# glennhickey/teHmm

Measured on AMD Instinct MI355X. Metric: genome positions/sec (Viterbi+posterior), 35 states x 10 tracks, higher is better.
Workload: dtype f64

## Files before the change

### tehmm_amd/csrc/tehmm_fused.hip.h

```cpp
#pragma once
#include "tehmm_lane.hip.h"

namespace tehmm {

template <int NT>
struct FusedGeom {
  static constexpr int KS = NT / 4;
  static constexpr int KSP = ((KS + 1) + 1) & ~1;
  static constexpr int RT = (NT + 15) / 16;
  static constexpr int SLICE_B = KSP * 8;
  static constexpr int ROW_D = 4 * KSP;
  static constexpr int ROW_D_LDS = 4 * KSP + 2;
};

#ifndef TEHMM_FUSED_2W
#define TEHMM_FUSED_2W 36
#endif
#define TEHMM_FUSED_BLKW 24
#ifndef TEHMM_FUSED_NSLOT_CAP
#define TEHMM_FUSED_NSLOT_CAP 64
#endif

struct FusedTab {
  const unsigned long long *rixx;
// ... 213 lines not shown
    const int blk = e / fo.SB, r = e - blk * fo.SB;
    unsigned long long *dst = rixx + ((tile * fo.NB + blk) * TEHMM_FUSED_BLKW + (int64_t)r * fo.FKW) * 16 + i16;
    for (int w = 0; w < fo.FKW; ++w) {
      unsigned long long word = 0;
      for (int b = 0; b < 4; ++b) {
        const int i = 4 * w + b;
        int v = 0;
        if (i < fo.K) {
          const int sym = orow[fo.order[i]];
          v = sym < fo.cnt[i] ? fo.base[i] + sym : (i < fo.n_glb ? fo.zero_glb : fo.zero_lds);
        }
        word |= (unsigned long long)(v & 0xffff) << (16 * b);
      }
      dst[(int64_t)w * 16] = word;
    }
  }
}


#define TEHMM_RIX_CB 4
#define TEHMM_RIX_STG 129
template <int FKW>
__global__ __launch_bounds__(256) void k_fused_rowindex(IntervalTab iv, LaneGeom lg, FusedOrder fo, const uint8_t *obs,
                                                        unsigned long long *rixx, int cps) {
  constexpr int SB = TEHMM_FUSED_BLKW / FKW, CB = TEHMM_RIX_CB, NS = CB * SB, STG = TEHMM_RIX_STG;
  __shared__ fused_u4 s_img[CB * 192];
  __shared__ fused_u4 s_slot[2 * TEHMM_FUSED_BLKW];
  __shared__ unsigned s_obs[16 * STG];
  __shared__ long long s_a0[16], s_T[16], s_row0[16];
  const int tid = threadIdx.x, lane = tid & 63, wv = tid >> 6;
  const int64_t tile = blockIdx.x;
  const int KPW = fo.KP >> 2;
  if (tid < 4 * TEHMM_FUSED_BLKW) {
    unsigned x = 0, y = 0;
    if (tid < fo.K) {
      const int cnt = fo.cnt[tid] < 256 ? fo.cnt[tid] : 256;
      x = (unsigned)fo.order[tid] | ((unsigned)cnt << 8);
      y = ((unsigned)fo.base[tid] & 0xffffu) | ((unsigned)(tid < fo.n_glb ? fo.zero_glb : fo.zero_lds) << 16);
    }
    unsigned *sl = (unsigned *)s_slot;
    sl[2 * tid] = x;
    sl[2 * tid + 1] = y;
  } else if (tid >= 128 && tid < 144) {
    const int64_t item = tile * 16 + (tid - 128);
    const bool valid = item < lg.n_items;
    const int id = valid ? lg.item_iv[item] : 0;
    s_a0[tid - 128] = (valid ? lg.item_t0[item] : 0) - fo.Wu;
    s_T[tid - 128] = iv.len[id];
    s_row0[tid - 128] = iv.pos0[id];
  }
  __syncthreads();
  const int nchunk = (fo.NB + CB - 1) / CB;
  const int c0 = blockIdx.y * cps, c1 = min(c0 + cps, nchunk);
  auto clampT = [](int64_t t, int64_t T) { return T > 0 ? (t < 0 ? 0 : (t >= T ? T - 1 : t)) : 0; };
  unsigned rr[4][2];
  auto load = [&](int c) {
#pragma unroll
    for (int j = 0; j < 4; ++j) {
      const int it = wv * 4 + j;
      const int64_t a = s_a0[it] + (int64_t)c * NS, T = s_T[it];
      const int64_t tf = clampT(a, T), tl = clampT(a + NS - 1, T);
      const int nd = (int)(tl - tf + 1) * KPW;
      const unsigned *src = (const unsigned *)obs + (s_row0[it] + tf) * KPW;
#pragma unroll
      for (int k = 0; k < 2; ++k) rr[j][k] = lane + 64 * k < nd ? src[lane + 64 * k] : 0u;
    }
  };
  const int i16 = tid & 15, q = tid >> 4;
  const int64_t my_a0 = s_a0[i16], my_T = s_T[i16];
  if (c0 < c1) load(c0);
  for (int c = c0; c < c1; ++c) {
#pragma unroll
    for (int j = 0; j < 4; ++j) {
#pragma unroll
      for (int k = 0; k < 2; ++k) s_obs[(wv * 4 + j) * STG + lane + 64 * k] = rr[j][k];
    }
    __syncthreads();
    if (c + 1 < c1) load(c + 1);
    const int64_t a = my_a0 + (int64_t)c * NS;
    int lo = 0, hi = 0, off = 0;
    if (my_T > 0) {
      const int64_t big = 1 << 30, l = -a, h = my_T - 1 - a;
      lo = (int)(l < -big ? -big : (l > big ? big : l));
      hi = (int)(h < -big ? -big : (h > big ? big : h));
      off = (int)(a - clampT(a, my_T));
    }
    const uint8_t *stage = (const uint8_t *)s_obs + i16 * (STG * 4);
#pragma unroll
    for (int jj = 0; jj < CB * TEHMM_FUSED_BLKW / 16; ++jj) {
      const int sw = q + 16 * jj, step = sw / FKW, w = sw - step * FKW;
      const uint8_t *row = stage + (min(max(step, lo), hi) + off) * fo.KP;
      const fused_u4 sa = s_slot[2 * w], sb = s_slot[2 * w + 1];
      const unsigned sx[4] = {sa.x, sa.z, sb.x, sb.z}, sy[4] = {sa.y, sa.w, sb.y, sb.w};
      unsigned long long word = 0;
#pragma unroll
      for (int b = 0; b < 4; ++b) {
        const unsigned sym = row[sx[b] & 0xffu];
        const unsigned v = sym < (sx[b] >> 8) ? (sy[b] & 0xffffu) + sym : sy[b] >> 16;
        word |= (unsigned long long)(v & 0xffffu) << (16 * b);
      }
      ((unsigned long long *)s_img)[tid + 256 * jj] = word;
    }
    __syncthreads();
    fused_u4 *dst = (fused_u4 *)rixx + (tile * fo.NB + (int64_t)c * CB) * 192;
#pragma unroll
    for (int jj = 0; jj < CB * 192 / 256; ++jj) {
      const int p = tid + 256 * jj;
      if (c * CB + p / 192 < fo.NB) dst[p] = s_img[p];
    }
  }
}

template <int NT, bool LOGDOM>
__global__ __launch_bounds__(256) __attribute__((amdgpu_waves_per_eu(NT <= TEHMM_FUSED_2W ? 2 : 1, NT <= TEHMM_FUSED_2W ? 2 : 1)))
void k_fused_fwd(IntervalTab iv, FusedTab ft, LaneGeom lg, int N, int CS, int Wu,
                 const double *__restrict__ tab , float *al32, double *chkf, double *pre,
                 double *end, double *slog32) {
  using G = FusedGeom<NT>;
  constexpr int KS = G::KS, RT = G::RT;
  extern __shared__ double fused_lds[];
  fused_stage<NT>(ft, fused_lds);
  __syncthreads();
  const int lane = threadIdx.x & 63;
  const int tile = blockIdx.x * 4 + (threadIdx.x >> 6);
  if (tile >= lg.n_groups * 4) return;
  const int L = lg.L;
  const int kq = lane >> 4;
  const int64_t item = (int64_t)tile * 16 + (lane & 15);
  const bool valid = item < lg.n_items;
  const int id = valid ? lg.item_iv[item] : 0;
  const int64_t t0 = valid ? lg.item_t0[item] : 0;
  const int64_t T = iv.len[id];
  const int64_t ct0 = (t0 / CS) * CS;
  const bool run = valid && ct0 + CS <= T && ct0 > 0;
  if (!__any(run)) return;
  double tf[RT][KS];
#pragma unroll
  for (int rt = 0; rt < RT; ++rt) {
#pragma unroll
    for (int s = 0; s < KS; ++s) {
      const int j = 16 * rt + (lane & 15), k = 4 * s + kq;
      tf[rt][s] = (j < NT) ? tab[k * NT + j] : 0.0;
    }
  }
  double v[KS];
#pragma unroll
  for (int s = 0; s < KS; ++s) v[s] = (kq + 4 * s < N) ? 1.0 / (double)N : 0.0;
  double slog = 0.0;
  auto vec_out = [&](double *dst) {
    const int64_t po = ((((item >> 6) * NT) + kq) << 6) + (item & 63);
#pragma unroll
    for (int s = 0; s < KS; ++s) dst[po + ((int64_t)(4 * s) << 6)] = v[s];
  };
  const double qnan = __longlong_as_double(0x7ff8000000000000LL);
  IndexWindow win;
  win.src = (const fused_u4 *)ft.rixx + (int64_t)tile * ft.NB * 192;
  win.lds_base = (unsigned)(size_t)(__attribute__((address_space(3))) const double *)fused_lds +
                 (unsigned)(ft.lds_rows * G::ROW_D_LDS * 8 + (threadIdx.x >> 6) * 2 * 3072);
  win.lane = lane;
  win.dir = 1;
  win.NB = ft.NB;
  win.start(0);
  double q[KS], ms;
  EmisStream<NT, LOGDOM> es(ft, fused_lds, win, kq);
  es.begin(0);
#pragma unroll
  for (int k = 0; k < KS; ++k) es.slot(k);
  es.finish(N, q, ms);
  const int E1 = ft.NB * ft.SB - 1;
  es.begin(min(1, E1));
  {
    float2 *ar = (float2 *)al32 + al32_index<NT>(lg, item, 0, kq) / 2;
#pragma unroll
    for (int p = 0; p < (KS + 1) / 2; ++p) ar[(int64_t)p * 64] = make_float2(0.f, 0.f);
  }
#ifdef TEHMM_STAMPS
  unsigned long long stq[4] = {0, 0, 0, 0}, stt = stamp_now();
#define FST(i) do { const unsigned long long n_ = stamp_now(); stq[i] += n_ - stt; stt = n_; } while (0)
#else
#define FST(i)
#endif
  for (int s = -Wu; s < L; ++s) {
    if (s == 0) {
      if (run) vec_out(pre);
      slog = 0.0;
    }
    FST(3);
    lane_d4 acc[RT];
#pragma unroll
    for (int rt = 0; rt < RT; ++rt) acc[rt] = (lane_d4){0.0, 0.0, 0.0, 0.0};
#pragma unroll
    for (int k = 0; k < KS; ++k) {
#pragma unroll
      for (int rt = 0; rt < RT; ++rt) acc[rt] = __builtin_amdgcn_mfma_f64_16x16x4f64(tf[rt][k], v[k], acc[rt], 0, 0, 0);
      es.slot(k);
      __builtin_amdgcn_sched_barrier(0);
    }
    FST(0);
    double qn[KS], msn = 0.0;
    es.finish(N, qn, msn);
    FST(1);
    double a[KS];
    double t = 0.0;
#pragma unroll
    for (int k = 0; k < KS; ++k) {
      a[k] = acc[k >> 2][k & 3] * q[k];
      t += a[k];
    }
    t = item_sum4(t);
    const int e = ((__double2hiint(t) >> 20) & 0x7ff) - 1022;
    const bool okrow = t > 1e-280 && t < INFINITY;
    const double scale = okrow ? __hiloint2double((1023 - e) << 20, 0) : qnan;
#pragma unroll
    for (int k = 0; k < KS; ++k) v[k] = a[k] * scale;
    slog += (double)e * 0.6931471805599453 + ms;
#pragma unroll
    for (int k = 0; k < KS; ++k) q[k] = qn[k];
    const double ms_now = ms;
    ms = msn;
    (void)ms_now;
    es.begin(min(s + 2 + Wu, E1));
    FST(2);
    {
      float2 *ar = (float2 *)al32 + al32_index<NT>(lg, item, s < 0 ? 0 : s, kq) / 2;
#pragma unroll
      for (int p = 0; p < (KS + 1) / 2; ++p)
        ar[(int64_t)p * 64] = run ? make_float2((float)v[2 * p], 2 * p + 1 < KS ? (float)v[2 * p + 1] : 0.f)
                                  : make_float2(0.f, 0.f);
    }
    if (s >= 0 && run) {
      if ((s & 31) == 31) {
        if (kq == 0) slog32[item * (L / 32) + (s >> 5)] = slog;
        if ((s & 63) == 31) {
          double *cr = chkf + (item * (L / 64) + (s >> 6)) * NT + kq;
#pragma unroll
          for (int k = 0; k < KS; ++k) cr[4 * k] = v[k];
        }
      }
    }
  }
  if (run) vec_out(end);
#ifdef TEHMM_STAMPS
  if (lane == 0 && blockIdx.x < 4096)
    for (int i = 0; i < 4; ++i) g_stamps[(blockIdx.x * 4 + (threadIdx.x >> 6)) * 4 + i] = stq[i];
#endif
#undef FST
}

template <int NT, bool LOGDOM, bool EPS, bool ESTEP = false>
__global__ __launch_bounds__(256) __attribute__((amdgpu_waves_per_eu(NT <= TEHMM_FUSED_2W ? 2 : 1, NT <= TEHMM_FUSED_2W ? 2 : 1)))
void k_fused_bwd(IntervalTab iv, FusedTab ft, LaneGeom lg, int N, int CS, int Wu,
                 const double *__restrict__ tab , const float *__restrict__ al32,
                 double *post, double *pre, double *end, double *chk, float *gam32 = nullptr, float *wz32 = nullptr,
                 double *sink = nullptr ) {
  using G = FusedGeom<NT>;
  constexpr int KS = G::KS, RT = G::RT;
  extern __shared__ double fused_lds[];
  fused_stage<NT>(ft, fused_lds);
  __syncthreads();
  const int lane = threadIdx.x & 63;
  const int tile = blockIdx.x * 4 + (threadIdx.x >> 6);
  if (tile >= lg.n_groups * 4) return;
  const int L = lg.L;
  const int kq = lane >> 4;
  const int64_t item = (int64_t)tile * 16 + (lane & 15);
  const bool valid = item < lg.n_items;
  const int id = valid ? lg.item_iv[item] : 0;
  const int64_t t0 = valid ? lg.item_t0[item] : 0;
  const int64_t T = iv.len[id];
  const int64_t ct0 = (t0 / CS) * CS;
  const bool run = valid && ct0 + CS <= T && ct0 + CS < T;
  if (!__any(run)) return;
  const int wu = !run ? 0 : (int)min((int64_t)Wu, T - (t0 + L));
  double tf[RT][KS];
#pragma unroll
  for (int rt = 0; rt < RT; ++rt) {
#pragma unroll
    for (int s = 0; s < KS; ++s) {
      const int j = 16 * rt + (lane & 15), k = 4 * s + kq;
      tf[rt][s] = (j < NT) ? tab[j * NT + k] : 0.0;
    }
  }
  double v[KS];
#pragma unroll
  for (int s = 0; s < KS; ++s) v[s] = 0.0;
  const int64_t prow0 = (iv.out0[id] + t0) * N;
  auto vec_out = [&](double *dst) {
    const int64_t po = ((((item >> 6) * NT) + kq) << 6) + (item & 63);
#pragma unroll
    for (int s = 0; s < KS; ++s) dst[po + ((int64_t)(4 * s) << 6)] = v[s];
  };
  const double eps = 1.1920928955078125e-07;
  const double inv_epsden = 1.0 / (1.0 + (double)N * eps);
  const double qnan = __longlong_as_double(0x7ff8000000000000LL);
  const int top = L + wu - 1;
  IndexWindow win;
  win.src = (const fused_u4 *)ft.rixx + (int64_t)tile * ft.NB * 192;
  win.lds_base = (unsigned)(size_t)(__attribute__((address_space(3))) const double *)fused_lds +
                 (unsigned)(ft.lds_rows * G::ROW_D_LDS * 8 + (threadIdx.x >> 6) * 2 * 3072);
  win.lane = lane;
  win.dir = -1;
  win.NB = ft.NB;
  win.start((L + 2 * Wu - 1) / ft.SB);
  typedef __attribute__((address_space(3))) double lds_f64;
  typedef __attribute__((address_space(3))) long long lds_i64;
  const unsigned ptile = (unsigned)(size_t)(__attribute__((address_space(3))) const double *)fused_lds +
                         (unsigned)(ft.lds_rows * G::ROW_D_LDS * 8 + 4 * 2 * 3072 + (threadIdx.x >> 6) * (16 * NT * 8 + 128));
  const unsigned pinfo = ptile + 16 * NT * 8;
  if (!ESTEP && kq == 0) *(lds_i64 *)(size_t)(pinfo + (lane & 15) * 8) = run ? (long long)prow0 : -1ll;
  double q[KS], ms;
  EmisStream<NT, LOGDOM> es(ft, fused_lds, win, kq);
  es.begin(L + 2 * Wu - 1);
#pragma unroll
  for (int k = 0; k < KS; ++k) es.slot(k);
  es.finish(N, q, ms);
  es.begin(max(L + 2 * Wu - 2, 0));
#ifdef TEHMM_STAMPS
  unsigned long long stq[4] = {0, 0, 0, 0}, stt = stamp_now();
#define FST(i) do { const unsigned long long n_ = stamp_now(); stq[i] += n_ - stt; stt = n_; } while (0)
#else
#define FST(i)
#endif
  for (int s = L + Wu - 1; s >= 0; --s) {
    if (s == L - 1 && run) vec_out(pre);
    FST(3);
    lane_d4 acc[RT];
#pragma unroll
    for (int rt = 0; rt < RT; ++rt) acc[rt] = (lane_d4){0.0, 0.0, 0.0, 0.0};
    float2 alp[(KS + 1) / 2];
    {
      const float2 *ar = (const float2 *)al32 + al32_index<NT>(lg, item, s < L ? s : L - 1, kq) / 2;
#pragma unroll
      for (int p = 0; p < (KS + 1) / 2; ++p) alp[p] = ar[(int64_t)p * 64];
    }
#pragma unroll
    for (int k = 0; k < KS; ++k) {
#pragma unroll
      for (int rt = 0; rt < RT; ++rt) acc[rt] = __builtin_amdgcn_mfma_f64_16x16x4f64(tf[rt][k], v[k], acc[rt], 0, 0, 0);
      es.slot(k);
      __builtin_amdgcn_sched_barrier(0);
    }
    FST(0);
#pragma unroll
    for (int p = 0; p < (KS + 1) / 2; ++p) asm volatile("" : "+v"(alp[p].x), "+v"(alp[p].y));
#pragma unroll
    for (int p = 0; p < (KS + 1) / 2; ++p) alp[p] = run ? alp[p] : make_float2(0.f, 0.f);
    double qn[KS], msn = 0.0;
    es.finish(N, qn, msn);
    FST(1);
    double t = 0.0;
#pragma unroll
    for (int k = 0; k < KS; ++k) t += acc[k >> 2][k & 3];
    t = item_sum4(t);
    const int e = ((__double2hiint(t) >> 20) & 0x7ff) - 1022;
    double bt[KS];
    const bool okrow = (s >= L && s >= top) || (t > 0.0 && t < INFINITY);
    const double scale = okrow ? __hiloint2double((1023 - e) << 20, 0) : qnan;
#pragma unroll
    for (int k = 0; k < KS; ++k) {
      bt[k] = acc[k >> 2][k & 3] * scale;
      if (s >= L && s == top) bt[k] = kq + 4 * k < N ? 1.0 : 0.0;
    }
    double g[KS];
    float wzf[ESTEP ? KS : 1];
#pragma unroll
    for (int k = 0; k < KS; ++k) g[k] = 0.0;
#pragma unroll
    for (int k = 0; k < (ESTEP ? KS : 1); ++k) wzf[k] = 0.f;
    if (s < L) {
      double gt = 0.0;
#pragma unroll
      for (int k = 0; k < KS; ++k) {
        g[k] = (double)((k & 1) ? alp[k >> 1].y : alp[k >> 1].x) * bt[k];
        gt += g[k];
      }
      gt = item_sum4(gt);
      const double inv = 1.0 / gt;
#pragma unroll
      for (int k = 0; k < KS; ++k) {
        g[k] *= inv;
        if (EPS) g[k] = (g[k] + eps) * inv_epsden;
      }
      if constexpr (ESTEP) {
        const double wzs = scale * inv;
#pragma unroll
        for (int k = 0; k < KS; ++k) wzf[k] = (float)(v[k] * wzs);
      }
#pragma unroll
      for (int k = 0; k < KS; ++k) v[k] = q[k] * bt[k];
#pragma unroll
      for (int k = 0; k < KS; ++k) q[k] = qn[k];
    }
    if (s >= L) {
#pragma unroll
      for (int k = 0; k < KS; ++k) v[k] = s > top ? 0.0 : q[k] * bt[k];
#pragma unroll
      for (int k = 0; k < KS; ++k) q[k] = qn[k];
    }
    es.begin(max(s - 2 + Wu, 0));
    {
      const bool off = s < L;
      if constexpr (ESTEP) {
        const int64_t ai = al32_index<NT>(lg, item, off ? s : L - 1, kq) / 2;
        float2 *gr = (float2 *)gam32 + ai, *wr = (float2 *)wz32 + ai;
#pragma unroll
        for (int p = 0; p < (KS + 1) / 2; ++p) {
          gr[(int64_t)p * 64] = run ? make_float2((float)g[2 * p], 2 * p + 1 < KS ? (float)g[2 * p + 1] : 0.f)
                                    : make_float2(0.f, 0.f);
          wr[(int64_t)p * 64] = run ? make_float2(wzf[2 * p], 2 * p + 1 < KS ? wzf[2 * p + 1] : 0.f)
                                    : make_float2(0.f, 0.f);
        }
      } else {
#pragma unroll
        for (int k = 0; k < KS; ++k) *(lds_f64 *)(size_t)(ptile + (unsigned)(((lane & 15) * NT + kq + 4 * k) * 8)) = g[k];
        int lane_v = lane;
        asm volatile("" : "+v"(lane_v));
        double *const snk = sink + ((int64_t)tile << 6) + lane;
        int offv = off ? 1 : 0;
        asm volatile("" : "+v"(offv));
        constexpr int NJ = (16 * NT + 63) / 64;
        double val[NJ];
        long long rbase[NJ];
#pragma unroll
        for (int j = 0; j < NJ; ++j) {
          const int e = 64 * j + lane_v;
          const int ec = (16 * NT % 64 == 0 || e < 16 * NT) ? e : 0;
          const int r = (ec * (65536 / NT + 1)) >> 16;
          val[j] = *(lds_f64 *)(size_t)(ptile + (unsigned)ec * 8u);
          rbase[j] = *(lds_i64 *)(size_t)(pinfo + (unsigned)r * 8u);
        }
#pragma unroll
        for (int j = 0; j < NJ; ++j) {
          const int e = 64 * j + lane_v;
          const int ec = (16 * NT % 64 == 0 || e < 16 * NT) ? e : 0;
          const int r = (ec * (65536 / NT + 1)) >> 16, c = ec - r * NT;
          const bool real = (offv != 0) & (rbase[j] >= 0) & (c < N) & (16 * NT % 64 == 0 || e < 16 * NT);
          double *dst = real ? post + (rbase[j] + (int64_t)s * N + c) : snk;
          asm volatile("" : "+v"(dst));
          *(__attribute__((address_space(1))) double *)dst = val[j];
        }
      }
      if (off && run) {
        if ((s & 63) == 31) {
          double *cr = chk + (item * (L / 64) + (s >> 6)) * NT + kq;
#pragma unroll
          for (int k = 0; k < KS; ++k) cr[4 * k] = bt[k];
        }
      }
    }
    FST(2);
    ms = msn;
  }
  (void)ms;
  if (run) vec_out(end);
#ifdef TEHMM_STAMPS
  if (lane == 0 && blockIdx.x < 4096)
    for (int i = 0; i < 4; ++i) g_stamps[4096 * 16 + (blockIdx.x * 4 + (threadIdx.x >> 6)) * 4 + i] = stq[i];
#endif
#undef FST
}

}
```

### tehmm_amd/csrc/tehmm_hip.hip

```cpp
#include <climits>
#include "tehmm_kernels.hip.h"
#include "tehmm_coop.hip.h"
#include "tehmm_lane.hip.h"
#include "tehmm_lane3.hip.h"
#include "tehmm_place.hip.h"
#include "tehmm_aux.hip.h"
#include "tehmm_fused.hip.h"
#include "tehmm_estep.hip.h"
#include "tehmm_wide_estep.hip.h"
#include "tehmm_wide.hip.h"
#include "tehmm_large.hip.h"
#include "tehmm_map.hip.h"
#include "tehmm_edist.hip.h"
#include "tehmm_segment.hip.h"
#include "tehmm_compare.hip.h"

#include <algorithm>
#include <atomic>
#include <cmath>
#include <cstdio>
#include <cstdlib>
#include <cstring>
#include <mutex>
#include <numeric>
// ... 4075 lines not shown
  const size_t na = (size_t)std::max(1, w.n_groups) * 64 * L * (NPW / 4) * 4;
  if (!w.GAM.p) {
    HIPCHK(w.GAM.alloc(na));
    HIPCHK(w.WZ.alloc(na));
    w.al_zeroed = false;
  }
  if (!w.al_zeroed) {
    HIPCHK(hipMemset(w.AL.p, 0, na * sizeof(float)));
    HIPCHK(hipMemset(w.GAM.p, 0, na * sizeof(float)));
    HIPCHK(hipMemset(w.WZ.p, 0, na * sizeof(float)));
    w.al_zeroed = true;
  }
  if (!b->fwd_lp.p || !b->dead.p) {
    HIPCHK(b->fwd_lp.alloc((size_t)b->n + 1));
    HIPCHK(b->dead.alloc((size_t)b->n + 1));
    if (!b->first_good.p) HIPCHK(b->first_good.alloc((size_t)b->n + 1));
  }
  if (w.rows_model != m->uid || w.rows_npw != NPW || !w.d_rows.p) {
    WideRows &wr = w.h_rows;
    WideLds &wl = w.h_lds;
    std::memset(&wl, 0, sizeof(wl));
    for (int i = 0; i < TEHMM_ESTEP_MAXRT * 16; ++i) { wr.info[i] = -1; wr.grow[i] = 0; }
    const int small = kn.estep_small;
    constexpr size_t kLdsCap = 150 * 1024;
    int big_rows = 0;
    for (int k = 0; k < m->K; ++k)
      if (m->rowcnt[k] > small) big_rows = std::max(big_rows, m->rowcnt[k]);
    w.lds_nsplit = (size_t)big_rows * NPW * 8 <= kLdsCap ? 1 : 2;
    int row = 0;
    wr.info[row++] = TEHMM_WIDE_ROW_START;
    wr.info[row++] = TEHMM_WIDE_ROW_DIAG;
    for (int k = 0; k < m->K; ++k) {
      const bool to_lds = m->rowcnt[k] > small && (size_t)m->rowcnt[k] * (NPW / w.lds_nsplit) * 8 <= kLdsCap;
      if (to_lds) {
        wl.col[wl.n_trk] = k;
        wl.rows[wl.n_trk] = m->rowcnt[k];
        wl.gbase[wl.n_trk] = m->rowbase[k];
        ++wl.n_trk;
        continue;
      }
      for (int sy = 0; sy < m->rowcnt[k]; ++sy, ++row) {
        if (row >= TEHMM_ESTEP_MAXRT * 16) return TEHMM_OK;
        wr.info[row] = (k & 255) | (sy << 8);
        wr.grow[row] = m->rowbase[k] + sy;
      }
    }
    wr.n_rt = (row + 15) / 16;
    HIPCHK(w.d_rows.upload(&wr, 1));
    HIPCHK(w.d_lds.upload(&wl, 1));
    w.rows_model = m->uid;
    w.rows_npw = NPW;
  }
  if (ratio && w.h_lds.n_trk > 0 && w.ratio_max <= 0.0) {
    if (!w.d_rmax.p) HIPCHK(w.d_rmax.alloc(1));
    HIPCHK(hipMemset(w.d_rmax.p, 0, sizeof(unsigned long long)));
    hipLaunchKernelGGL(k_ratio_max, dim3(grid_for(b->total_pad, 256, 2048)), dim3(256), 0, b->sP, (const double *)b->ratios.p,
                       b->total_pad, w.d_rmax.p);
    unsigned long long bits = 0;
    HIPCHK(hipMemcpyAsync(&bits, w.d_rmax.p, sizeof(bits), hipMemcpyDeviceToHost, b->sP));
    HIPCHK(hipStreamSynchronize(b->sP));
    double rmax = 0.0;
    std::memcpy(&rmax, &bits, sizeof(rmax));
    if (!(rmax < 1e12)) return TEHMM_OK;
    w.ratio_max = std::max(rmax, 1e-300);
  }
  IntervalTab iv;
  EmisTab em;
  fill_tabs(m, b, iv, em, ratio);
  const LaneGeom lg = wide_lane_geom(w);
  hipStream_t st = b->sP;
  b->tnames.clear();
  b->tpairs.clear();
  b->tms.clear();
  (void)hipEventRecord(b->ev[10], st);
  HIPCHK(hipMemsetAsync(w.flags.p, 0, 4 * sizeof(int), st));
  launch_wide_emis(b, m, iv, em, lg, ratio ? 3 : 2, nullptr, st);
  (void)hipEventRecord(b->ev[12], st);
  (void)hipEventRecord(b->ev[9], st);
  if (int rc = wide_post_attempt(b, m, iv, kn, wide_first_warmup(w, m, kn, false), st, b->ev[8], true)) return rc;
  WideRetries re = {b->ev[9], b->ev[6], 1};
  bool verified = false;
  if (int rc = wide_verdict(b, m, iv, kn, st, b->ev[8], true, &re, &verified)) return rc;
  if (!verified) return TEHMM_OK;
  int rcr = TEHMM_OK;
  nt_dispatch_of<TEHMM_WIDE_ESTEP_WIDTHS>(NPW, [&](auto npw) { rcr = launch_wide_estep_reduce<npw>(b, m, iv, lg, ratio, kn, dev_stats, st); });
  if (rcr) return rcr;
  (void)hipEventRecord(b->ev[7], st);
  HIPCHK(hipGetLastError());
  HIPCHK(hipStreamSynchronize(st));
  static const struct { const char *name; int a, b2; } stages[] = {
      {"estep_emission_rows", 10, 12}, {"estep_forward_pass", 9, 8}, {"estep_backward_pass", 8, 6}, {"estep_reduce", 6, 7}};
  for (const auto &sg : stages) {
    float ms = 0.f;
    (void)hipEventElapsedTime(&ms, b->ev[sg.a], b->ev[sg.b2]);
    b->tnames.push_back(sg.name);
    b->tms.push_back((double)ms);
  }
  b->tnames.push_back("count:wide_estep_attempts");
  b->tms.push_back((double)re.attempts);
  b->tnames.push_back("count:wide_estep_warmup");
  b->tms.push_back((double)w.wu_ok);
  std::vector<double> lp((size_t)b->n);
  HIPCHK(hipMemcpy(lp.data(), b->fwd_lp.p, (size_t)b->n * sizeof(double), hipMemcpyDeviceToHost));
  double lp_total = 0.0;
  for (int id = 0; id < b->n; ++id) {
    if (b->h_len[(size_t)id] <= 0) continue;
    lp_total += lp[(size_t)id];
    b->h_fwd_lp[(size_t)id] = lp[(size_t)id];
  }
  *lp_out = lp_total;
  *dead_out = 0;
  *done = true;
  return TEHMM_OK;
}

static int estep_accumulate(tehmm_model_t *m, tehmm_batch_t *b, int use_ratios, double *dev_stats, double *lp_out,
                            int *dead_out) {
#ifdef TEHMM_DEV_NT
  if (m->N < 64 && m->NP != TEHMM_DEV_NT)
    return fail(TEHMM_ERR_UNSUPPORTED, "development build: fused kernels exist for one padded state count only");
#endif
  *lp_out = 0.0;
  *dead_out = 0;
  b->h_fwd_lp.assign((size_t)b->n, 0.0);
  if (b->n == 0 || b->total == 0) return TEHMM_OK;
  const bool ratio = use_ratios && b->has_ratios;
  const int N = m->N, NP = m->NP;
  {
    bool done = false;
    const EvalKnobs kn = read_eval_knobs();
    const bool wide_first = kn.estep_wide == 2;
    if (!ratio && N < 64 && !wide_first) {
      int rcf = estep_fused(m, b, kn, dev_stats, lp_out, dead_out, &done);
      if (rcf) return rcf;
      if (done) return TEHMM_OK;
    }
    int rcw = estep_wide(m, b, kn, ratio, dev_stats, lp_out, dead_out, &done);
    if (rcw) return rcw;
    if (done) return TEHMM_OK;
    if (N >= 64)
      return fail(TEHMM_ERR_UNSUPPORTED, "E-step at N >= 64: the item-parallel passes do not apply to this batch (impossible "
                                         "emission rows, links that do not verify, or a batch below 1024 rows): use the array-level path");
  }
  size_t free_b = 0, total_b = 0;
  (void)dev_mem_info(&free_b, &total_b);
  int64_t budget_bytes = (int64_t)((double)(free_b + (size_t)b->ew.rows_cap * (24 * N + 4)) * 0.4);
  if (budget_bytes < (4ll << 30)) budget_bytes = 4ll << 30;
  const int64_t budget_rows = std::max<int64_t>(budget_bytes / (24 * N + 4), 1);
  EstepWork &w = b->ew;
  if (w.N != N) {
    w.alpha.release();
    w.rows_cap = 0;
    w.N = N;
  }
  w.start = dev_stats + stats_off_start();
  w.C = dev_stats + stats_off_C(NP);
  w.D = dev_stats + stats_off_D(NP);
  w.stat = dev_stats + stats_off_stat(NP);
  IntervalTab iv;
  EmisTab em;
  fill_tabs(m, b, iv, em, ratio);
  double lp_total = 0.0;
  int dead_any = 0;
  size_t pos_in_order = 0;
  while (pos_in_order < (size_t)b->n) {
    std::vector<int> g_order;
    std::vector<int64_t> grow0((size_t)b->n, 0);
    std::vector<int> chunk_iv;
    std::vector<int64_t> chunk_t0;
    int64_t rows = 0;
    while (pos_in_order < (size_t)b->n) {
      const int id = b->h_order[pos_in_order];
      const int64_t T = b->h_len[id];
      if (!g_order.empty() && rows + T > budget_rows) break;
      g_order.push_back(id);
      grow0[id] = rows;
      for (int64_t t0 = 0; t0 < T; t0 += kEstepChunk) {
        chunk_iv.push_back(id);
        chunk_t0.push_back(t0);
      }
      rows += T;
      ++pos_in_order;
    }
    if (rows == 0) continue;
    if (rows > w.rows_cap) {
      HIPCHK(w.alpha.alloc((size_t)rows * N + 1));
      HIPCHK(w.beta.alloc((size_t)rows * N + 1));
      HIPCHK(w.wrows.alloc((size_t)rows * N + 1));
      HIPCHK(w.escale.alloc((size_t)rows + 1));
      w.rows_cap = rows;
    }
    if (b->n > w.n_cap) {
      HIPCHK(w.fwd_lp.alloc((size_t)b->n + 1));
      HIPCHK(w.dead.alloc((size_t)b->n + 1));
      w.n_cap = b->n;
    }
    HIPCHK(hipMemset(w.dead.p, 0, (size_t)(b->n + 1) * sizeof(int)));
    HIPCHK(hipMemset(w.escale.p, 0, ((size_t)rows + 1) * sizeof(int)));
    HIPCHK(w.order.upload(g_order.data(), g_order.size()));
    HIPCHK(w.grow0.upload(grow0.data(), grow0.size()));
    HIPCHK(w.chunk_iv.upload(chunk_iv.data(), chunk_iv.size()));
    HIPCHK(w.chunk_t0.upload(chunk_t0.data(), chunk_t0.size()));
    IntervalTab giv = iv;
    giv.order = w.order.p;
    giv.out0 = w.grow0.p;
    const int n_iv = (int)g_order.size(), n_chunks = (int)chunk_iv.size();
    nt_dispatch(m->NP, [&](auto nt) { launch_estep<nt>(m, giv, em, ratio, n_iv, n_chunks, w, b->ratios.p, b->sP); });
    HIPCHK(hipGetLastError());
    HIPCHK(hipStreamSynchronize(b->sP));
    std::vector<double> lp((size_t)b->n);
    std::vector<int> dead((size_t)b->n);
    HIPCHK(hipMemcpy(lp.data(), w.fwd_lp.p, (size_t)b->n * sizeof(double), hipMemcpyDeviceToHost));
    HIPCHK(hipMemcpy(dead.data(), w.dead.p, (size_t)b->n * sizeof(int), hipMemcpyDeviceToHost));
    for (int id : g_order) {
      lp_total += lp[(size_t)id];
      dead_any |= dead[(size_t)id];
      b->h_fwd_lp[(size_t)id] = dead[(size_t)id] ? std::nan("") : lp[(size_t)id];
    }
  }
  *lp_out = lp_total;
  *dead_out = dead_any;
  return TEHMM_OK;
}

int64_t tehmm_model_stats_size(const tehmm_model_t *m) {
  if (m && m->large) return fail(TEHMM_ERR_UNSUPPORTED, "tehmm_model_stats_size: no device-resident statistics for N > 128");
  return m ? stats_size(m->NP, m->R) : 0;
}

int tehmm_estep_batch_device(tehmm_model_t *m, tehmm_batch_t *b, int use_ratios, double *dev_stats,
                             double *logprob_sum) {
  if (!m || !b || !dev_stats || !logprob_sum)
    return fail(TEHMM_ERR_ARG, "tehmm_estep_batch_device: NULL argument");
  if (m->K != b->K) return fail(TEHMM_ERR_ARG, "tehmm_estep_batch_device: model/batch track count differ");
  if (m->N > 128)
    return fail(TEHMM_ERR_UNSUPPORTED, "tehmm_estep_batch_device: N > 128 (the E-step of such a model runs on the "
                                       "array-level entry points)");
  double lp = 0.0;
  int dead = 0;
  int rc = estep_accumulate(m, b, use_ratios, dev_stats, &lp, &dead);
  if (rc) return rc;
  const double nan = std::nan("");
  double head[2];
  HIPCHK(hipMemcpy(head, dev_stats, sizeof(head), hipMemcpyDeviceToHost));
  head[0] += dead ? nan : lp;
  head[1] += (double)b->n;
  HIPCHK(hipMemcpy(dev_stats, head, sizeof(head), hipMemcpyHostToDevice));
  if (dead) {
    std::vector<double> bad((size_t)stats_size(m->NP, m->R), nan);
    bad[1] = head[1];
    HIPCHK(hipMemcpy(dev_stats, bad.data(), bad.size() * sizeof(double), hipMemcpyHostToDevice));
  }
  *logprob_sum = dead ? nan : lp;
  return TEHMM_OK;
}

int tehmm_estep_batch(tehmm_model_t *m, tehmm_batch_t *b, int use_ratios, double *start,
                      double *trans, double *obsStats, double *logprob_sum) {
  if (!m || !b || !start || !trans || !obsStats || !logprob_sum)
    return fail(TEHMM_ERR_ARG, "tehmm_estep_batch: NULL argument");
  if (m->K != b->K) return fail(TEHMM_ERR_ARG, "tehmm_estep_batch: model/batch track count differ");
  if (m->N > 128)
    return fail(TEHMM_ERR_UNSUPPORTED, "tehmm_estep_batch: N > 128 (the E-step of such a model runs on the array-level "
                                       "entry points)");
  *logprob_sum = 0.0;
  if (b->n == 0 || b->total == 0) return TEHMM_OK;
  const int N = m->N, NP = m->NP, K = m->K, S = m->S;
  EstepWork &w = b->ew;
  const size_t ssz = (size_t)stats_size(NP, m->R);
  HIPCHK(w.statbuf.ensure(ssz));
  HIPCHK(hipMemset(w.statbuf.p, 0, ssz * sizeof(double)));
  double lp_total = 0.0;
  int dead_any = 0;
  int rc = estep_accumulate(m, b, use_ratios, w.statbuf.p, &lp_total, &dead_any);
  if (rc) return rc;
  std::vector<double> hs(ssz);
  HIPCHK(hipMemcpy(hs.data(), w.statbuf.p, ssz * sizeof(double), hipMemcpyDeviceToHost));
  const double *hS = hs.data() + stats_off_start(), *hC = hs.data() + stats_off_C(NP),
               *hD = hs.data() + stats_off_D(NP), *hst = hs.data() + stats_off_stat(NP);
  const double nan = std::nan("");
  const double invN = 1.0 / (double)N;
  for (int i = 0; i < N; ++i) {
    start[i] += dead_any ? nan : hS[i];
    for (int j = 0; j < N; ++j) {
      double v = std::exp(m->h_lt[(size_t)i * N + j]) * hC[(size_t)i * NP + j];
      if (i == j) v += hD[i];
      trans[(size_t)i * N + j] += dead_any ? nan : v * invN;
    }
  }
  for (int k = 0; k < K; ++k)
    for (int s2 = 0; s2 < m->rowcnt[k]; ++s2)
      for (int j = 0; j < N; ++j)
        obsStats[((size_t)k * N + j) * S + s2] += dead_any ? nan : hst[(size_t)(m->rowbase[k] + s2) * NP + j];
  *logprob_sum = dead_any ? nan : lp_total;
  return TEHMM_OK;
}

#include "tehmm_aux_host.inc"
#include "tehmm_segment_host.inc"
#include "tehmm_compare_host.inc"

int tehmm_debug_read_stamps(unsigned long long *out, int n) {
#ifdef TEHMM_STAMPS
  if (!out || n <= 0 || n > 2 * 4096 * 16) return fail(TEHMM_ERR_ARG, "tehmm_debug_read_stamps: bad argument");
  HIPCHK(hipMemcpyFromSymbol(out, HIP_SYMBOL(g_stamps), (size_t)n * sizeof(unsigned long long)));
  return TEHMM_OK;
#else
  (void)out; (void)n;
  return fail(TEHMM_ERR_UNSUPPORTED, "tehmm_debug_read_stamps: library built without -DTEHMM_STAMPS");
#endif
}

int tehmm_debug_read_rowindex(tehmm_batch_t *b, unsigned long long *out, int64_t max_words, int64_t *n_words) {
  if (!b || !n_words || max_words < 0 || (max_words > 0 && !out))
    return fail(TEHMM_ERR_ARG, "tehmm_debug_read_rowindex: bad argument");
  if (!b->lw.rix.p || !b->lw.rix_model || !b->lw.rix_words)
    return fail(TEHMM_ERR_ARG, "tehmm_debug_read_rowindex: the batch holds no index records");
  if (b->sV) HIPCHK(hipStreamSynchronize(b->sV));
  if (b->sP) HIPCHK(hipStreamSynchronize(b->sP));
  if (b->sB) HIPCHK(hipStreamSynchronize(b->sB));
  *n_words = (int64_t)b->lw.rix_words;
  if (*n_words <= max_words)
    HIPCHK(hipMemcpy(out, b->lw.rix.p, b->lw.rix_words * sizeof(unsigned long long), hipMemcpyDeviceToHost));
  return TEHMM_OK;
}
```

### tehmm_amd/csrc/tehmm_kernels.hip.h

```cpp
#pragma once
#include <hip/hip_runtime.h>
#include <stdint.h>

#define TEHMM_WAVE 64
#ifndef TEHMM_PRIO_HI
#define TEHMM_PRIO_HI 3
#define TEHMM_PRIO_LO 2
#endif
#define TEHMM_MAX_TRACKS 128
#define TEHMM_PB 16
#define TEHMM_TB_CHUNK 256

namespace tehmm {

#ifdef TEHMM_STAMPS
__device__ unsigned long long g_stamps[2 * 4096 * 16];
__device__ __forceinline__ unsigned long long stamp_now() {
  unsigned long long t;
  asm volatile("s_memtime %0\n\ts_waitcnt lgkmcnt(0)" : "=s"(t)::"memory");
  return t;
}
#define ST_DECL unsigned long long st_a = 0, st_b = 0, st_c = 0, st_t0 = 0, st_t1 = 0
#define ST_BEGIN st_t0 = stamp_now()
#define ST_ADD(acc) do { st_t1 = stamp_now(); acc += st_t1 - st_t0; st_t0 = st_t1; } while (0)
#define ST_FLUSH(w_)                                                                        \
  do {                                                                                      \
    if ((threadIdx.x & 63) == 0 && blockIdx.x < 4096) {                                     \
      g_stamps[(blockIdx.x * 4 + (w_)) * 4 + 0] = st_a;                                     \
      g_stamps[(blockIdx.x * 4 + (w_)) * 4 + 1] = st_b;                                     \
      g_stamps[(blockIdx.x * 4 + (w_)) * 4 + 2] = st_c;                                     \
    }                                                                                       \
  } while (0)
#else
#define ST_DECL
#define ST_BEGIN
#define ST_ADD(acc)
#define ST_FLUSH(w_)
#endif

struct EmisTab {
  const uint32_t *obs32;
  const double *tab;
  const double *ratios;
  double normalize;
  int K, KPW, NP;
  int rowbase[TEHMM_MAX_TRACKS];
  int rowcnt[TEHMM_MAX_TRACKS];
  int ldsbase[TEHMM_MAX_TRACKS];
  int lds_rows;
  const double *ltab_src;
  int zero_row, lds_zero;
};

struct IntervalTab {
  const int *order;
  const int64_t *pos0;
  const int64_t *len;
  const int64_t *out0;
  int n;
};

__device__ __forceinline__ double wave_max_f64(double v) {
#pragma unroll
  for (int o = 32; o > 0; o >>= 1) v = fmax(v, __shfl_xor(v, o));
  return v;
}
__device__ __forceinline__ double wave_sum_f64(double v) {
#pragma unroll
  for (int o = 32; o > 0; o >>= 1) v += __shfl_xor(v, o);
  return v;
}
__device__ __forceinline__ int wave_max_i32(int v) {
#pragma unroll
  for (int o = 32; o > 0; o >>= 1) v = max(v, __shfl_xor(v, o));
  return v;
}
__device__ __forceinline__ int exp_of(double a) {
  return ((__double2hiint(a) >> 20) & 0x7ff) - 1022;
}

template <int SPL>
__device__ __forceinline__ void emis_log(const EmisTab &e, int64_t gpos, int lane, int N,
                                         double (&x)[SPL]) {
  const uint32_t *row = e.obs32 + gpos * e.KPW;
#pragma unroll
  for (int s = 0; s < SPL; ++s) x[s] = 0.0;
  for (int k = 0; k < e.K; ++k) {
    uint32_t w = row[k >> 2];
    int sym = (int)((w >> ((k & 3) * 8)) & 0xffu);
    const int trow = sym < e.rowcnt[k] ? e.rowbase[k] + sym : e.zero_row;
    const double *tr = e.tab + (int64_t)trow * e.NP;
#pragma unroll
    for (int s = 0; s < SPL; ++s) {
      int j = lane + TEHMM_WAVE * s;
      if (j < N) x[s] += tr[j];
    }
  }
#pragma unroll
  for (int s = 0; s < SPL; ++s) x[s] *= e.normalize;
  if (e.ratios) {
    double r = e.ratios[gpos];
#pragma unroll
    for (int s = 0; s < SPL; ++s) x[s] *= r;
  }
}

template <int SPL>
__device__ __forceinline__ double row_max(const double (&x)[SPL], int lane, int N) {
  double m = -INFINITY;
#pragma unroll
  for (int s = 0; s < SPL; ++s)
    if (lane + TEHMM_WAVE * s < N) m = fmax(m, x[s]);
  return wave_max_f64(m);
}

__global__ void k_repack_obs(int n, const int64_t *out0, const int64_t *pos0, const int64_t *len,
                             int K, int KP, const uint8_t *src, uint8_t *dst,
                             const double *rsrc, double *rdst) {
  int iv = blockIdx.y;
  if (iv >= n) return;
  int64_t T = len[iv];
  const uint8_t *s = src + out0[iv] * K;
  uint8_t *d = dst + pos0[iv] * KP;
  for (int64_t idx = blockIdx.x * (int64_t)blockDim.x + threadIdx.x; idx < T * KP;
       idx += (int64_t)gridDim.x * blockDim.x) {
    int64_t t = idx / KP;
    int k = (int)(idx - t * KP);
    d[idx] = k < K ? s[t * K + k] : (uint8_t)0;
  }
  if (rsrc) {
    for (int64_t t = blockIdx.x * (int64_t)blockDim.x + threadIdx.x; t < T;
         t += (int64_t)gridDim.x * blockDim.x)
      rdst[pos0[iv] + t] = rsrc[out0[iv] + t];
  }
}

template <typename ObsT>
__global__ void k_emission(int64_t T, int K, int N, int S, const ObsT *obs, const double *lp,
                           double normalize, const double *ratios, double *out,
                           unsigned long long *first_good) {
  int64_t total = T * N;
  for (int64_t idx = blockIdx.x * (int64_t)blockDim.x + threadIdx.x; idx < total;
       idx += (int64_t)gridDim.x * blockDim.x) {
    int64_t t = idx / N;
    int j = (int)(idx - t * N);
    double x = 0.0;
    for (int k = 0; k < K; ++k) {
      int64_t sym = (int64_t)obs[t * K + k];
      if (sym >= 0 && sym < S) x += lp[((int64_t)k * N + j) * S + sym];
    }
    x *= normalize;
    if (ratios) x *= ratios[t];
    out[idx] = x;
    if (x > -1e20) atomicMin(first_good, (unsigned long long)t);
  }
}
__global__ void k_emission_fix(int64_t T, int N, double *out, const unsigned long long *first_good) {
  unsigned long long fg = *first_good;
  int64_t rows = fg > (unsigned long long)T ? T : (int64_t)fg;
  for (int64_t idx = blockIdx.x * (int64_t)blockDim.x + threadIdx.x; idx < rows * N;
       idx += (int64_t)gridDim.x * blockDim.x)
    out[idx] = 0.0;
}

__global__ __launch_bounds__(64) void k_forward_log(int64_t T, int N, const double *pi,
                                                    const double *lt, const double *frame,
                                                    const double *ratios, double *fwd) {
  extern __shared__ double sm[];
  double *prev = sm, *next = sm + N;
  const int lane = threadIdx.x;
  const bool hasr = ratios != nullptr;
  {
    double r0 = hasr ? ratios[0] : 0.0;
    for (int j = lane; j < N; j += TEHMM_WAVE) {
      double a = pi[j] + frame[j];
      if (hasr && r0 > 1.) a += lt[(int64_t)j * N + j] * (r0 - 1.);
      fwd[j] = a;
      prev[j] = a;
    }
  }
  __syncthreads();
  for (int64_t t = 1; t < T; ++t) {
    double rt = hasr ? ratios[t] : 0.0;
    bool rr = hasr && rt > 1.;
    for (int j = lane; j < N; j += TEHMM_WAVE) {
      double add = rr ? lt[(int64_t)j * N + j] * (rt - 1.) : 0.0;
      double vmax = -INFINITY;
      for (int i = 0; i < N; ++i) {
        double w = prev[i] + lt[(int64_t)i * N + j];
        if (rr) w += add;
        if (w > vmax) vmax = w;
      }
      double ps = 0.0;
      for (int i = 0; i < N; ++i) {
        double w = prev[i] + lt[(int64_t)i * N + j];
        if (rr) w += add;
        ps += exp(w - vmax);
      }
      double v = log(ps) + vmax + frame[t * N + j];
      if (v <= -1e200) v = -INFINITY;
      fwd[t * N + j] = v;
      next[j] = v;
    }
    __syncthreads();
    double *tmp = prev; prev = next; next = tmp;
  }
}

__global__ __launch_bounds__(64) void k_backward_log(int64_t T, int N, const double *lt,
                                                     const double *frame, const double *ratios,
                                                     double *bwd) {
  extern __shared__ double sm[];
  double *prev = sm, *next = sm + N;
  double *fb = sm + 2 * N;
  const int lane = threadIdx.x;
  const bool hasr = ratios != nullptr;
  {
    double v = log(1. / (double)N);
    for (int j = lane; j < N; j += TEHMM_WAVE) {
      bwd[(T - 1) * N + j] = v;
      prev[j] = v;
    }
  }
  __syncthreads();
  for (int64_t t = T - 2; t >= 0; --t) {
    double rt = hasr ? ratios[t + 1] : 0.0;
    bool rr = hasr && rt > 1.;
    for (int j = lane; j < N; j += TEHMM_WAVE) fb[j] = frame[(t + 1) * N + j];
    __syncthreads();
    for (int i = lane; i < N; i += TEHMM_WAVE) {
      double vmax = -INFINITY;
      for (int j = 0; j < N; ++j) {
        double w = lt[(int64_t)i * N + j] + fb[j] + prev[j];
        if (rr) w += lt[(int64_t)j * N + j] * (rt - 1.);
        if (w > vmax) vmax = w;
      }
      double ps = 0.0;
      for (int j = 0; j < N; ++j) {
        double w = lt[(int64_t)i * N + j] + fb[j] + prev[j];
        if (rr) w += lt[(int64_t)j * N + j] * (rt - 1.);
        ps += exp(w - vmax);
      }
      double v = log(ps) + vmax;
      if (v <= -1e200) v = -INFINITY;
      bwd[t * N + i] = v;
      next[i] = v;
    }
    __syncthreads();
    double *tmp = prev; prev = next; next = tmp;
  }
}

__global__ void k_xi_logsum(int64_t T, int N, const double *fwd, const double *lt,
                            const double *bwd, const double *frame, double logprob,
                            const double *ratios, double *out) {
  int idx = blockIdx.x * blockDim.x + threadIdx.x;
  if (idx >= N * N) return;
  int i = idx / N, j = idx - i * N;
  const bool hasr = ratios != nullptr;
  double lij = lt[idx], ljj = lt[(int64_t)j * N + j];
  double mx = -INFINITY;
  for (int64_t t = 0; t < T - 1; ++t) {
    double x = fwd[t * N + i] + lij + frame[(t + 1) * N + j] + bwd[(t + 1) * N + j] - logprob;
    if (hasr && ratios[t + 1] > 1.) {
      x += ljj * (ratios[t + 1] - 1.);
      if (i == j) {
        double y = fwd[(t + 1) * N + i] + bwd[(t + 1) * N + j] + log(ratios[t + 1] - 1.) - logprob;
        if (y > mx) mx = y;
      }
    }
    if (x > mx) mx = x;
  }
  double acc = out[idx];
  for (int64_t t = 0; t < T - 1; ++t) {
    double x = fwd[t * N + i] + lij + frame[(t + 1) * N + j] + bwd[(t + 1) * N + j] - logprob;
    if (hasr && ratios[t + 1] > 1.) {
      x += ljj * (ratios[t + 1] - 1.);
      if (i == j) {
        double y = fwd[(t + 1) * N + i] + bwd[(t + 1) * N + j] + log(ratios[t + 1] - 1.) - logprob;
        acc += exp(y - mx);
      }
    }
    acc += exp(x - mx);
  }
  out[idx] = log(acc) + mx;
}

template <typename ObsT>
__global__ void k_accumulate_obs(int64_t T, int K, int N, int S, const ObsT *obs,
                                 double *obsStats, const double *post, const double *ratios) {
  int idx = blockIdx.x * blockDim.x + threadIdx.x;
  if (idx >= K * N) return;
  int k = idx / N, j = idx - k * N;
  double *row = obsStats + (int64_t)idx * S;
  for (int64_t t = 0; t < T; ++t) {
    double p = post[t * N + j];
    if (ratios) p *= ratios[t];
    const int64_t sym = (int64_t)obs[t * K + k];
    if (sym >= 0 && sym < S) row[sym] += p;
  }
}

template <typename ObsT>
__global__ void k_update_counts(int n_iv, const int64_t *iv_start, const int64_t *iv_end,
                                const int32_t *iv_state, int K, int N, int S, const ObsT *obs,
                                double *obsStats, const double *ratios) {
  const int k = blockIdx.x, state = blockIdx.y;
  for (int sym = threadIdx.x; sym < S; sym += blockDim.x) {
    double acc = obsStats[((int64_t)k * N + state) * S + sym];
    bool touched = false;
    for (int i = 0; i < n_iv; ++i) {
      if (iv_state[i] != state) continue;
      for (int64_t pos = iv_start[i]; pos < iv_end[i]; ++pos) {
        if ((int64_t)obs[pos * K + k] == (int64_t)sym) {
          acc += ratios ? ratios[pos] : 1.0;
          touched = true;
        }
      }
    }
// ... 1101 lines not shown
```

Baseline: 1.545 billion.

## Defer posterior stores and interleave them with next step's MFMA slots

In the non-E-step, linear-domain fused backward kernel, the posterior tile written to LDS at each step is no longer scattered to global memory straight away. It is read back and stored during the next step's MFMA/emission slot loop, using row base addresses and a run mask kept in scalar registers, and a final flush runs after the loop. The aim is to hide global store and address-computation latency behind the matrix work on the serial recurrence path. In exchange it holds 16 row pointers in registers, which may raise register pressure, and the timing-stamp instrumentation is widened to five buckets.

```diff
diff --git a/tehmm_amd/csrc/tehmm_fused.hip.h b/tehmm_amd/csrc/tehmm_fused.hip.h
--- a/tehmm_amd/csrc/tehmm_fused.hip.h
+++ b/tehmm_amd/csrc/tehmm_fused.hip.h
@@ -539,12 +539,51 @@
   win.dir = -1;
   win.NB = ft.NB;
   win.start((L + 2 * Wu - 1) / ft.SB);
+  constexpr bool DEFER = !ESTEP && !LOGDOM;
   typedef __attribute__((address_space(3))) double lds_f64;
   typedef __attribute__((address_space(3))) long long lds_i64;
   const unsigned ptile = (unsigned)(size_t)(__attribute__((address_space(3))) const double *)fused_lds +
                          (unsigned)(ft.lds_rows * G::ROW_D_LDS * 8 + 4 * 2 * 3072 + (threadIdx.x >> 6) * (16 * NT * 8 + 128));
   const unsigned pinfo = ptile + 16 * NT * 8;
   if (!ESTEP && kq == 0) *(lds_i64 *)(size_t)(pinfo + (lane & 15) * 8) = run ? (long long)prow0 : -1ll;
+  unsigned long long prow[16];
+  unsigned prun = 0;
+  unsigned long long psink = 0;
+  const int pcol = !DEFER ? 0 : lane < N ? lane : lane % N;
+  const unsigned pread = ptile + (unsigned)pcol * 8u;
+  if constexpr (DEFER) {
+#pragma unroll
+    for (int r = 0; r < 16; ++r) {
+      const long long rb = *(lds_i64 *)(size_t)(pinfo + (unsigned)r * 8u);
+      const unsigned rlo = (unsigned)rb, rhi = (unsigned)((unsigned long long)rb >> 32);
+      const unsigned lo = NT <= TEHMM_FUSED_2W ? __builtin_amdgcn_readfirstlane(rlo) : rlo;
+      const unsigned hi = NT <= TEHMM_FUSED_2W ? __builtin_amdgcn_readfirstlane(rhi) : rhi;
+      const unsigned long long rbu = ((unsigned long long)hi << 32) | lo;
+      prow[r] = (unsigned long long)(size_t)post + rbu * 8ull;
+      prun |= (int)__builtin_amdgcn_readfirstlane(rhi) >= 0 ? 1u << r : 0u;
+    }
+    psink = (unsigned long long)(size_t)(sink + ((int64_t)__builtin_amdgcn_readfirstlane(tile) << 6));
+  }
+  constexpr int RPS = (16 + KS - 1) / KS;
+  double pval[RPS];
+#pragma unroll
+  for (int i = 0; i < RPS; ++i) pval[i] = 0.0;
+  auto post_slot = [&](int k, unsigned mk, int so) {
+    const unsigned voff = (unsigned)(so + pcol) * 8u;
+    const unsigned long long sadj = psink - (unsigned long long)so * 8ull;
+    if (k > 0) {
+#pragma unroll
+      for (int r = 16 * (k - 1) / KS; r < 16 * k / KS; ++r) {
+        const unsigned long long base = ((mk >> r) & 1u) ? prow[r] : sadj;
+        *(__attribute__((address_space(1))) double *)(size_t)(base + voff) = pval[r - 16 * (k - 1) / KS];
+      }
+    }
+    if (k < KS) {
+#pragma unroll
+      for (int r = 16 * k / KS; r < 16 * (k + 1) / KS; ++r)
+        pval[r - 16 * k / KS] = *(lds_f64 *)(size_t)(pread + (unsigned)(r * NT * 8));
+    }
+  };
   double q[KS], ms;
   EmisStream<NT, LOGDOM> es(ft, fused_lds, win, kq);
   es.begin(L + 2 * Wu - 1);
@@ -553,7 +592,7 @@
   es.finish(N, q, ms);
   es.begin(max(L + 2 * Wu - 2, 0));
 #ifdef TEHMM_STAMPS
-  unsigned long long stq[4] = {0, 0, 0, 0}, stt = stamp_now();
+  unsigned long long stq[5] = {0, 0, 0, 0, 0}, stt = stamp_now();
 #define FST(i) do { const unsigned long long n_ = stamp_now(); stq[i] += n_ - stt; stt = n_; } while (0)
 #else
 #define FST(i)
@@ -570,11 +609,20 @@
 #pragma unroll
       for (int p = 0; p < (KS + 1) / 2; ++p) alp[p] = ar[(int64_t)p * 64];
     }
+    unsigned pmk = s + 1 < L ? prun : 0u;
+    if constexpr (DEFER) asm volatile("" : "+s"(pmk));
+    const int pso = (s + 1) * N;
+    (void)pmk, (void)pso;
 #pragma unroll
     for (int k = 0; k < KS; ++k) {
 #pragma unroll
       for (int rt = 0; rt < RT; ++rt) acc[rt] = __builtin_amdgcn_mfma_f64_16x16x4f64(tf[rt][k], v[k], acc[rt], 0, 0, 0);
       es.slot(k);
+      if constexpr (DEFER) post_slot(k, pmk, pso);
+      __builtin_amdgcn_sched_barrier(0);
+    }
+    if constexpr (DEFER) {
+      post_slot(KS, pmk, pso);
       __builtin_amdgcn_sched_barrier(0);
     }
     FST(0);
@@ -635,6 +683,7 @@
       for (int k = 0; k < KS; ++k) q[k] = qn[k];
     }
     es.begin(max(s - 2 + Wu, 0));
+    FST(2);
     {
       const bool off = s < L;
       if constexpr (ESTEP) {
@@ -650,31 +699,33 @@
       } else {
 #pragma unroll
         for (int k = 0; k < KS; ++k) *(lds_f64 *)(size_t)(ptile + (unsigned)(((lane & 15) * NT + kq + 4 * k) * 8)) = g[k];
-        int lane_v = lane;
-        asm volatile("" : "+v"(lane_v));
-        double *const snk = sink + ((int64_t)tile << 6) + lane;
-        int offv = off ? 1 : 0;
-        asm volatile("" : "+v"(offv));
-        constexpr int NJ = (16 * NT + 63) / 64;
-        double val[NJ];
-        long long rbase[NJ];
-#pragma unroll
-        for (int j = 0; j < NJ; ++j) {
-          const int e = 64 * j + lane_v;
-          const int ec = (16 * NT % 64 == 0 || e < 16 * NT) ? e : 0;
-          const int r = (ec * (65536 / NT + 1)) >> 16;
-          val[j] = *(lds_f64 *)(size_t)(ptile + (unsigned)ec * 8u);
-          rbase[j] = *(lds_i64 *)(size_t)(pinfo + (unsigned)r * 8u);
-        }
-#pragma unroll
-        for (int j = 0; j < NJ; ++j) {
-          const int e = 64 * j + lane_v;
-          const int ec = (16 * NT % 64 == 0 || e < 16 * NT) ? e : 0;
-          const int r = (ec * (65536 / NT + 1)) >> 16, c = ec - r * NT;
-          const bool real = (offv != 0) & (rbase[j] >= 0) & (c < N) & (16 * NT % 64 == 0 || e < 16 * NT);
-          double *dst = real ? post + (rbase[j] + (int64_t)s * N + c) : snk;
-          asm volatile("" : "+v"(dst));
-          *(__attribute__((address_space(1))) double *)dst = val[j];
+        if constexpr (!DEFER) {
+          int lane_v = lane;
+          asm volatile("" : "+v"(lane_v));
+          double *const snk = sink + ((int64_t)tile << 6) + lane;
+          int offv = off ? 1 : 0;
+          asm volatile("" : "+v"(offv));
+          constexpr int NJ = (16 * NT + 63) / 64;
+          double val[NJ];
+          long long rbase[NJ];
+#pragma unroll
+          for (int j = 0; j < NJ; ++j) {
+            const int e = 64 * j + lane_v;
+            const int ec = (16 * NT % 64 == 0 || e < 16 * NT) ? e : 0;
+            const int r = (ec * (65536 / NT + 1)) >> 16;
+            val[j] = *(lds_f64 *)(size_t)(ptile + (unsigned)ec * 8u);
+            rbase[j] = *(lds_i64 *)(size_t)(pinfo + (unsigned)r * 8u);
+          }
+#pragma unroll
+          for (int j = 0; j < NJ; ++j) {
+            const int e = 64 * j + lane_v;
+            const int ec = (16 * NT % 64 == 0 || e < 16 * NT) ? e : 0;
+            const int r = (ec * (65536 / NT + 1)) >> 16, c = ec - r * NT;
+            const bool real = (offv != 0) & (rbase[j] >= 0) & (c < N) & (16 * NT % 64 == 0 || e < 16 * NT);
+            double *dst = real ? post + (rbase[j] + (int64_t)s * N + c) : snk;
+            asm volatile("" : "+v"(dst));
+            *(__attribute__((address_space(1))) double *)dst = val[j];
+          }
         }
       }
       if (off && run) {
@@ -685,14 +736,20 @@
         }
       }
     }
-    FST(2);
+    FST(4);
     ms = msn;
   }
   (void)ms;
+  if constexpr (DEFER) {
+    unsigned pmk = L > 0 ? prun : 0u;
+    asm volatile("" : "+s"(pmk));
+#pragma unroll
+    for (int k = 0; k <= KS; ++k) post_slot(k, pmk, 0);
+  }
   if (run) vec_out(end);
 #ifdef TEHMM_STAMPS
   if (lane == 0 && blockIdx.x < 4096)
-    for (int i = 0; i < 4; ++i) g_stamps[4096 * 16 + (blockIdx.x * 4 + (threadIdx.x >> 6)) * 4 + i] = stq[i];
+    for (int i = 0; i < 5; ++i) g_stamps[4096 * 16 + (blockIdx.x * 4 + (threadIdx.x >> 6)) * 8 + i] = stq[i];
 #endif
 #undef FST
 }
diff --git a/tehmm_amd/csrc/tehmm_hip.hip b/tehmm_amd/csrc/tehmm_hip.hip
--- a/tehmm_amd/csrc/tehmm_hip.hip
+++ b/tehmm_amd/csrc/tehmm_hip.hip
@@ -4401,7 +4401,7 @@
 
 int tehmm_debug_read_stamps(unsigned long long *out, int n) {
 #ifdef TEHMM_STAMPS
-  if (!out || n <= 0 || n > 2 * 4096 * 16) return fail(TEHMM_ERR_ARG, "tehmm_debug_read_stamps: bad argument");
+  if (!out || n <= 0 || (size_t)n > sizeof(g_stamps) / sizeof(g_stamps[0])) return fail(TEHMM_ERR_ARG, "tehmm_debug_read_stamps: bad argument");
   HIPCHK(hipMemcpyFromSymbol(out, HIP_SYMBOL(g_stamps), (size_t)n * sizeof(unsigned long long)));
   return TEHMM_OK;
 #else
diff --git a/tehmm_amd/csrc/tehmm_kernels.hip.h b/tehmm_amd/csrc/tehmm_kernels.hip.h
--- a/tehmm_amd/csrc/tehmm_kernels.hip.h
+++ b/tehmm_amd/csrc/tehmm_kernels.hip.h
@@ -14,7 +14,7 @@
 namespace tehmm {
 
 #ifdef TEHMM_STAMPS
-__device__ unsigned long long g_stamps[2 * 4096 * 16];
+__device__ unsigned long long g_stamps[3 * 4096 * 16];
 __device__ __forceinline__ unsigned long long stamp_now() {
   unsigned long long t;
   asm volatile("s_memtime %0\n\ts_waitcnt lgkmcnt(0)" : "=s"(t)::"memory");
```

New measurement: 1.573 billion (median of 6 runs). 1.02x the previous value.
